# dmosopt/dmosopt

Measured on NVIDIA H100. Metric: candidate-evals/sec (GP+sort+HV) pop=65536 dim=30 obj=3, higher is better.
Workload: dtype f64 results; GP variance contraction in split-fp16 wgmma with fp32 accumulation (precision=auto: calibrated against the float64 path, 0 of 65535 rows of the last step recomputed in float64); ranks on u32 ids

## Files before the change

dmosopt_b200/csrc/gp_tensor.cu:

```cuda
#include <cuda.h>
#include <cuda_fp16.h>
#include <cudaTypedefs.h>
#include <stdlib.h>

#include "gp.cuh"

namespace {

constexpr int TN = 256;
constexpr int TMV = 128;
constexpr int TK = 32;
constexpr int UK = 16;
constexpr int STAGES = 4;
constexpr int A_BYTES = TMV * TK * 2;
constexpr int B_BYTES = TN * TK * 2;
constexpr int STAGE_BYTES = 2 * A_BYTES + 2 * B_BYTES;
constexpr size_t GEMM_SMEM = (size_t)STAGES * STAGE_BYTES + 1024 + 256;
constexpr int NTHREADS = 384;

__device__ __forceinline__ uint32_t smem_u32(const void* p) { return (uint32_t)__cvta_generic_to_shared(p); }

__device__ __forceinline__ void mbar_init(uint64_t* bar, uint32_t count) {
  asm volatile("mbarrier.init.shared::cta.b64 [%0], %1;" ::"r"(smem_u32(bar)), "r"(count) : "memory");
}
__device__ __forceinline__ void mbar_arrive(uint64_t* bar) {
  asm volatile("mbarrier.arrive.shared::cta.b64 _, [%0];" ::"r"(smem_u32(bar)) : "memory");
}
__device__ __forceinline__ void mbar_expect_tx(uint64_t* bar, uint32_t bytes) {
  asm volatile("mbarrier.arrive.expect_tx.shared::cta.b64 _, [%0], %1;" ::"r"(smem_u32(bar)), "r"(bytes) : "memory");
}
__device__ __forceinline__ bool mbar_try_wait(uint64_t* bar, uint32_t parity) {
  uint32_t ok;
  asm volatile(
      "{\n"
      ".reg .pred p;\n"
      "mbarrier.try_wait.parity.shared::cta.b64 p, [%1], %2;\n"
      "selp.u32 %0, 1, 0, p;\n"
      "}\n"
      : "=r"(ok)
      : "r"(smem_u32(bar)), "r"(parity)
      : "memory");
  return ok != 0;
}
__device__ __forceinline__ void mbar_wait(uint64_t* bar, uint32_t parity, volatile int* abort_flag) {
  uint32_t spins = 0;
  while (!mbar_try_wait(bar, parity)) {
    if ((++spins & 0x3FFu) == 0u) {
      if (*abort_flag) return;
      if (spins > (1u << 22)) {
        *abort_flag = 1;
        return;
      }
    }
  }
}

__device__ __forceinline__ void tma_load_2d(const CUtensorMap* map, uint64_t* bar, void* dst, int c0, int c1) {
  asm volatile(
      "cp.async.bulk.tensor.2d.shared::cluster.global.tile.mbarrier::complete_tx::bytes [%0], [%1, {%3, %4}], [%2];" ::"r"(
          smem_u32(dst)),
      "l"(map), "r"(smem_u32(bar)), "r"(c0), "r"(c1)
      : "memory");
}

__device__ __forceinline__ uint64_t make_sdesc64(uint32_t smem_addr) {
  return (uint64_t)((smem_addr >> 4) & 0x3FFFu) | (1ull << 16) | ((uint64_t)(512 >> 4) << 32) | (2ull << 62);
}

__device__ __forceinline__ void wgmma_fence() { asm volatile("wgmma.fence.sync.aligned;" ::: "memory"); }
__device__ __forceinline__ void wgmma_commit() { asm volatile("wgmma.commit_group.sync.aligned;" ::: "memory"); }
template <int N>
__device__ __forceinline__ void wgmma_wait() {
  asm volatile("wgmma.wait_group.sync.aligned %0;" ::"n"(N) : "memory");
}

__device__ __forceinline__ void wgmma_f16_m64n256(float (&d)[128], uint64_t adesc, uint64_t bdesc, uint32_t accumulate) {
  asm volatile(
      "{\n"
      ".reg .pred p;\n"
      "setp.ne.b32 p, %130, 0;\n"
      "wgmma.mma_async.sync.aligned.m64n256k16.f32.f16.f16 "
      "{"
      "%0, %1, %2, %3, %4, %5, %6, %7, %8, %9, %10, %11, %12, %13, %14, %15, "
      "%16, %17, %18, %19, %20, %21, %22, %23, %24, %25, %26, %27, %28, %29, %30, %31, "
      "%32, %33, %34, %35, %36, %37, %38, %39, %40, %41, %42, %43, %44, %45, %46, %47, "
      "%48, %49, %50, %51, %52, %53, %54, %55, %56, %57, %58, %59, %60, %61, %62, %63, "
      "%64, %65, %66, %67, %68, %69, %70, %71, %72, %73, %74, %75, %76, %77, %78, %79, "
      "%80, %81, %82, %83, %84, %85, %86, %87, %88, %89, %90, %91, %92, %93, %94, %95, "
      "%96, %97, %98, %99, %100, %101, %102, %103, %104, %105, %106, %107, %108, %109, %110, %111, "
      "%112, %113, %114, %115, %116, %117, %118, %119, %120, %121, %122, %123, %124, %125, %126, %127}, "
      "%128, %129, p, 1, 1, 0, 0;\n"
      "}\n"
      : "+f"(d[0]), "+f"(d[1]), "+f"(d[2]), "+f"(d[3]), "+f"(d[4]), "+f"(d[5]), "+f"(d[6]), "+f"(d[7]),
        "+f"(d[8]), "+f"(d[9]), "+f"(d[10]), "+f"(d[11]), "+f"(d[12]), "+f"(d[13]), "+f"(d[14]), "+f"(d[15]),
        "+f"(d[16]), "+f"(d[17]), "+f"(d[18]), "+f"(d[19]), "+f"(d[20]), "+f"(d[21]), "+f"(d[22]), "+f"(d[23]),
        "+f"(d[24]), "+f"(d[25]), "+f"(d[26]), "+f"(d[27]), "+f"(d[28]), "+f"(d[29]), "+f"(d[30]), "+f"(d[31]),
        "+f"(d[32]), "+f"(d[33]), "+f"(d[34]), "+f"(d[35]), "+f"(d[36]), "+f"(d[37]), "+f"(d[38]), "+f"(d[39]),
        "+f"(d[40]), "+f"(d[41]), "+f"(d[42]), "+f"(d[43]), "+f"(d[44]), "+f"(d[45]), "+f"(d[46]), "+f"(d[47]),
        "+f"(d[48]), "+f"(d[49]), "+f"(d[50]), "+f"(d[51]), "+f"(d[52]), "+f"(d[53]), "+f"(d[54]), "+f"(d[55]),
        "+f"(d[56]), "+f"(d[57]), "+f"(d[58]), "+f"(d[59]), "+f"(d[60]), "+f"(d[61]), "+f"(d[62]), "+f"(d[63]),
        "+f"(d[64]), "+f"(d[65]), "+f"(d[66]), "+f"(d[67]), "+f"(d[68]), "+f"(d[69]), "+f"(d[70]), "+f"(d[71]),
        "+f"(d[72]), "+f"(d[73]), "+f"(d[74]), "+f"(d[75]), "+f"(d[76]), "+f"(d[77]), "+f"(d[78]), "+f"(d[79]),
        "+f"(d[80]), "+f"(d[81]), "+f"(d[82]), "+f"(d[83]), "+f"(d[84]), "+f"(d[85]), "+f"(d[86]), "+f"(d[87]),
        "+f"(d[88]), "+f"(d[89]), "+f"(d[90]), "+f"(d[91]), "+f"(d[92]), "+f"(d[93]), "+f"(d[94]), "+f"(d[95]),
        "+f"(d[96]), "+f"(d[97]), "+f"(d[98]), "+f"(d[99]), "+f"(d[100]), "+f"(d[101]), "+f"(d[102]), "+f"(d[103]),
        "+f"(d[104]), "+f"(d[105]), "+f"(d[106]), "+f"(d[107]), "+f"(d[108]), "+f"(d[109]), "+f"(d[110]), "+f"(d[111]),
        "+f"(d[112]), "+f"(d[113]), "+f"(d[114]), "+f"(d[115]), "+f"(d[116]), "+f"(d[117]), "+f"(d[118]), "+f"(d[119]),
        "+f"(d[120]), "+f"(d[121]), "+f"(d[122]), "+f"(d[123]), "+f"(d[124]), "+f"(d[125]), "+f"(d[126]), "+f"(d[127])
      : "l"(adesc), "l"(bdesc), "r"(accumulate)
      : "memory");
}

struct GemmParams {
  int M, n_pb, n_jt, n_q;
  int64_t k_rows, l_rows;
  const float* inv_scale;
  double* vnorm;
  int64_t vn_ld;
  int* abort_flag;
};

__device__ __forceinline__ int item_blocks(const GemmParams& p, int q) { return q == p.n_jt - 1 - q ? 1 : 2; }
__device__ __forceinline__ int item_row_block(const GemmParams& p, int q, int s) { return s ? p.n_jt - 1 - q : q; }

__global__ void __launch_bounds__(NTHREADS, 1)
    gp_var_wgmma_kernel(const __grid_constant__ CUtensorMap map_kh, const __grid_constant__ CUtensorMap map_kl,
                        const __grid_constant__ CUtensorMap map_lh, const __grid_constant__ CUtensorMap map_ll,
                        const GemmParams prm) {
  extern __shared__ uint8_t smem_raw[];
  uint8_t* tiles = (uint8_t*)(((uintptr_t)smem_raw + 1023) & ~(uintptr_t)1023);
  uint64_t* bars = (uint64_t*)(tiles + (size_t)STAGES * STAGE_BYTES);
  uint64_t* full = bars;
  uint64_t* empty = bars + STAGES;
  volatile int* abort_flag = prm.abort_flag;
  const int warp = threadIdx.x >> 5, lane = threadIdx.x & 31;

  if (threadIdx.x == 0) {
    for (int s = 0; s < STAGES; ++s) {
      mbar_init(&full[s], 1);
      mbar_init(&empty[s], 8);
    }
    asm volatile("fence.mbarrier_init.release.cluster;" ::: "memory");
  }
  __syncthreads();
  const int per_m = prm.n_pb * prm.n_q;
  const int n_work = prm.M * per_m;

  if (warp >= 8) {
    asm volatile("setmaxnreg.dec.sync.aligned.u32 40;\n" ::: "memory");
    if (warp == 8 && lane == 0) {
      uint32_t stage = 0, phase = 0;
      for (int w = blockIdx.x; w < n_work; w += gridDim.x) {
        const int m = w / per_m, r = w - m * per_m;
        const int pb = r / prm.n_q, q = r - pb * prm.n_q;
        const int a_row = (int)(m * prm.k_rows + (int64_t)pb * TMV);
        const int nb = item_blocks(prm, q);
        for (int s = 0; s < nb; ++s) {
          const int jt = item_row_block(prm, q, s);
          const int b_row = (int)(m * prm.l_rows + (int64_t)jt * TN);
          const int nkc = (jt + 1) * (TN / TK);
          for (int kc = 0; kc < nkc; ++kc) {
            mbar_wait(&empty[stage], phase ^ 1u, abort_flag);
            uint8_t* st = tiles + (size_t)stage * STAGE_BYTES;
            mbar_expect_tx(&full[stage], STAGE_BYTES);
            tma_load_2d(&map_kh, &full[stage], st, kc * TK, a_row);
            tma_load_2d(&map_kl, &full[stage], st + A_BYTES, kc * TK, a_row);
            tma_load_2d(&map_lh, &full[stage], st + 2 * A_BYTES, kc * TK, b_row);
            tma_load_2d(&map_ll, &full[stage], st + 2 * A_BYTES + B_BYTES, kc * TK, b_row);
            if (++stage == STAGES) {
              stage = 0;
              phase ^= 1u;
            }
          }
        }
      }
    }
    return;
  }

  asm volatile("setmaxnreg.inc.sync.aligned.u32 232;\n" ::: "memory");
  const int wg = warp >> 2;
  const int row0 = wg * 64 + (warp & 3) * 16 + (lane >> 2);
  const int col0 = 2 * (lane & 3);
  float acc[128];
  uint32_t stage = 0, phase = 0;
  for (int w = blockIdx.x; w < n_work; w += gridDim.x) {
    const int m = w / per_m, r = w - m * per_m;
    const int pb = r / prm.n_q, q = r - pb * prm.n_q;
    const float* isc = prm.inv_scale + (int64_t)m * prm.l_rows;
    double total0 = 0.0, total1 = 0.0;
    const int nb = item_blocks(prm, q);
    for (int s = 0; s < nb; ++s) {
      const int jt = item_row_block(prm, q, s);
      const int nkc = (jt + 1) * (TN / TK);
      uint32_t prev = 0;
      for (int kc = 0; kc < nkc; ++kc) {
        mbar_wait(&full[stage], phase, abort_flag);
        const uint32_t sa = smem_u32(tiles + (size_t)stage * STAGE_BYTES);
        const uint32_t a_off = wg * (64 * TK * 2);
        const uint64_t a_hi = make_sdesc64(sa + a_off), a_lo = make_sdesc64(sa + A_BYTES + a_off);
        const uint64_t b_hi = make_sdesc64(sa + 2 * A_BYTES), b_lo = make_sdesc64(sa + 2 * A_BYTES + B_BYTES);
        wgmma_fence();
#pragma unroll
        for (int ks = 0; ks < TK / UK; ++ks) {
          const uint64_t adv = (uint64_t)((ks * UK * 2) >> 4);
          wgmma_f16_m64n256(acc, a_hi + adv, b_hi + adv, (kc | ks) ? 1u : 0u);
          wgmma_f16_m64n256(acc, a_hi + adv, b_lo + adv, 1u);
          wgmma_f16_m64n256(acc, a_lo + adv, b_hi + adv, 1u);
        }
        wgmma_commit();
        if (kc > 0) {
          wgmma_wait<1>();
          if (lane == 0) mbar_arrive(&empty[prev]);
        }
        prev = stage;
        if (++stage == STAGES) {
          stage = 0;
          phase ^= 1u;
        }
      }
      wgmma_wait<0>();
      if (lane == 0) mbar_arrive(&empty[prev]);
      const float* sc = isc + jt * TN + col0;
#pragma unroll
      for (int g = 0; g < TN / 32; ++g) {
        float p0[4] = {0.f, 0.f, 0.f, 0.f}, p1[4] = {0.f, 0.f, 0.f, 0.f};
#pragma unroll
        for (int u = 0; u < 4; ++u) {
          const int i = 4 * g + u;
          const float2 sv = __ldg(reinterpret_cast<const float2*>(sc + 8 * i));
          const float t00 = acc[4 * i] * sv.x, t01 = acc[4 * i + 1] * sv.y;
          const float t10 = acc[4 * i + 2] * sv.x, t11 = acc[4 * i + 3] * sv.y;
          p0[u] = fmaf(t01, t01, t00 * t00);
          p1[u] = fmaf(t11, t11, t10 * t10);
        }
        total0 += ((double)p0[0] + (double)p0[1]) + ((double)p0[2] + (double)p0[3]);
        total1 += ((double)p1[0] + (double)p1[1]) + ((double)p1[2] + (double)p1[3]);
      }
    }
#pragma unroll
    for (int o = 1; o < 4; o <<= 1) {
      total0 += __shfl_xor_sync(0xffffffffu, total0, o);
      total1 += __shfl_xor_sync(0xffffffffu, total1, o);
    }
    if ((lane & 3) == 0) {
      const int64_t o = ((int64_t)q * prm.M + m) * prm.vn_ld + (int64_t)pb * TMV + row0;
      prm.vnorm[o] = total0;
      prm.vnorm[o + 8] = total1;
    }
  }
}

__global__ void split_linv_kernel(const double* __restrict__ Linv, int64_t Npad, const int* __restrict__ k_exp,
                                  uint16_t* __restrict__ Lh, uint16_t* __restrict__ Ll, float* __restrict__ inv_scale) {
  const int64_t row = blockIdx.x;
  const int g = (int)(row / Npad);
  const double* src = Linv + row * Npad;
  __shared__ double red[256];
  double mx = 0.0;
  for (int64_t k = threadIdx.x; k < Npad; k += blockDim.x) mx = fmax(mx, fabs(src[k]));
  red[threadIdx.x] = mx;
  __syncthreads();
  for (int o = 128; o > 0; o >>= 1) {
    if (threadIdx.x < o) red[threadIdx.x] = fmax(red[threadIdx.x], red[threadIdx.x + o]);
    __syncthreads();
  }
  mx = red[0];
  int e = 0;
  if (mx > 0.0) e = 13 - ilogb(mx);
  const double s = scalbn(1.0, e);
  for (int64_t k = threadIdx.x; k < Npad; k += blockDim.x) {
    const float x = (float)(src[k] * s);
    const __half h = __float2half_rn(x);
    const __half l = __float2half_rn(x - __half2float(h));
    Lh[row * Npad + k] = __half_as_ushort(h);
    Ll[row * Npad + k] = __half_as_ushort(l);
  }
  if (threadIdx.x == 0) inv_scale[row] = (mx > 0.0) ? (float)scalbn(1.0, -e - k_exp[g]) : 0.f;
}

constexpr int KT_TN = 128, KT_TP = 32;

__device__ __forceinline__ float stationary_f(float s2, int kind) {
  if (kind == DMO_KERNEL_MATERN52) {
    float r;
    asm("sqrt.approx.ftz.f32 %0, %1;" : "=f"(r) : "f"(s2));
    const float K = r * 2.2360679774997896f;
    return fmaf(K, fmaf(K, 1.0f / 3.0f, 1.0f), 1.0f) * __expf(-K);
  }
  return __expf(-0.5f * s2);
}

__device__ __forceinline__ float2 fadd2(float2 a, float2 b) { return make_float2(__fadd_rn(a.x, b.x), __fadd_rn(a.y, b.y)); }
__device__ __forceinline__ float2 fmul2(float2 a, float2 b) { return make_float2(__fmul_rn(a.x, b.x), __fmul_rn(a.y, b.y)); }
__device__ __forceinline__ float2 ffma2(float2 a, float2 b, float2 c) {
  return make_float2(__fmaf_rn(a.x, b.x, c.x), __fmaf_rn(a.y, b.y, c.y));
}

__device__ __forceinline__ float2 stationary2_f(float2 s2, int kind) {
  float2 e;
  if (kind == DMO_KERNEL_MATERN52) {
    float2 r;
    asm("sqrt.approx.ftz.f32 %0, %1;" : "=f"(r.x) : "f"(s2.x));
    asm("sqrt.approx.ftz.f32 %0, %1;" : "=f"(r.y) : "f"(s2.y));
    const float2 K = fmul2(r, make_float2(2.2360679774997896f, 2.2360679774997896f));
    const float2 one = make_float2(1.0f, 1.0f);
    const float2 p = ffma2(K, ffma2(K, make_float2(1.0f / 3.0f, 1.0f / 3.0f), one), one);
    const float2 t = fmul2(K, make_float2(-1.4426950408889634f, -1.4426950408889634f));
    asm("ex2.approx.ftz.f32 %0, %1;" : "=f"(e.x) : "f"(t.x));
    asm("ex2.approx.ftz.f32 %0, %1;" : "=f"(e.y) : "f"(t.y));
    return fmul2(p, e);
  }
  const float2 t = fmul2(s2, make_float2(-0.5f * 1.4426950408889634f, -0.5f * 1.4426950408889634f));
  asm("ex2.approx.ftz.f32 %0, %1;" : "=f"(e.x) : "f"(t.x));
  asm("ex2.approx.ftz.f32 %0, %1;" : "=f"(e.y) : "f"(t.y));
  return e;
}

template <bool ISO, int DMAX>
__global__ void __launch_bounds__(KT_TN)
    kstar_tensor_kernel(const double* __restrict__ Xn, int64_t P, int64_t p_base, int64_t Pcpad,
                        const double* __restrict__ Xt, int64_t N, int d, int M, int kind,
                        const double* __restrict__ inv_ls, const double* __restrict__ constant,
                        const int* __restrict__ k_exp, int64_t ldk, int64_t plane, uint16_t* __restrict__ Kh,
                        uint16_t* __restrict__ Kl) {
  extern __shared__ __align__(16) float sxf[];
  float* s_il = sxf + KT_TP * DMAX;
  float* s_c = s_il + M * DMAX;
  const int64_t n0 = ((int64_t)blockIdx.x * KT_TN + threadIdx.x) * 2;
  const int64_t pt0 = (int64_t)blockIdx.y * KT_TP;
  for (int t = threadIdx.x; t < KT_TP * DMAX; t += KT_TN) {
    const int64_t p = p_base + pt0 + t / DMAX;
    const int j = t % DMAX;
    sxf[t] = (p < P && j < d) ? (float)Xn[p * d + j] : 0.f;
  }
  for (int t = threadIdx.x; t < M * DMAX; t += KT_TN) {
    const int m = t / DMAX, j = t % DMAX;
    s_il[t] = j < d ? (float)inv_ls[m * d + j] : 0.f;
  }
  if (threadIdx.x < M) s_c[threadIdx.x] = scalbnf((float)constant[threadIdx.x], k_exp[threadIdx.x]);
  float2 xa[DMAX / 2], xb[DMAX / 2];
#pragma unroll
  for (int j = 0; j < DMAX / 2; ++j) {
    const int j0 = 2 * j, j1 = 2 * j + 1;
    xa[j] = make_float2((j0 < d && n0 < N) ? (float)Xt[n0 * d + j0] : 0.f, (j1 < d && n0 < N) ? (float)Xt[n0 * d + j1] : 0.f);
    xb[j] = make_float2((j0 < d && n0 + 1 < N) ? (float)Xt[(n0 + 1) * d + j0] : 0.f,
                        (j1 < d && n0 + 1 < N) ? (float)Xt[(n0 + 1) * d + j1] : 0.f);
  }
  __syncthreads();
  const bool live_a = n0 < N, live_b = n0 + 1 < N;
  uint32_t* Kh32 = reinterpret_cast<uint32_t*>(Kh);
  uint32_t* Kl32 = reinterpret_cast<uint32_t*>(Kl);
  for (int q = 0; q < KT_TP; ++q) {
    const int64_t pl = pt0 + q;
    if (pl >= Pcpad || n0 >= ldk) break;
    const float4* xc = reinterpret_cast<const float4*>(sxf + q * DMAX);
    float sa = 0.f, sb = 0.f;
    if (ISO) {
      float2 acc_a0 = make_float2(0.f, 0.f), acc_a1 = acc_a0, acc_b0 = acc_a0, acc_b1 = acc_a0;
#pragma unroll
      for (int j = 0; j < DMAX / 4; ++j) {
        const float4 c = xc[j];
        const float2 c01 = make_float2(c.x, c.y), c23 = make_float2(c.z, c.w);
        const float2 da0 = fadd2(c01, make_float2(-xa[2 * j].x, -xa[2 * j].y));
        const float2 db0 = fadd2(c01, make_float2(-xb[2 * j].x, -xb[2 * j].y));
        const float2 da1 = fadd2(c23, make_float2(-xa[2 * j + 1].x, -xa[2 * j + 1].y));
        const float2 db1 = fadd2(c23, make_float2(-xb[2 * j + 1].x, -xb[2 * j + 1].y));
        acc_a0 = ffma2(da0, da0, acc_a0);
        acc_b0 = ffma2(db0, db0, acc_b0);
        acc_a1 = ffma2(da1, da1, acc_a1);
        acc_b1 = ffma2(db1, db1, acc_b1);
      }
      sa = (acc_a0.x + acc_a0.y) + (acc_a1.x + acc_a1.y);
      sb = (acc_b0.x + acc_b0.y) + (acc_b1.x + acc_b1.y);
    }
    for (int m = 0; m < M; ++m) {
      float2 rr;
      if (ISO) {
        const float il = s_il[m * DMAX];
        const float il2 = il * il;
        rr = fmul2(make_float2(sa, sb), make_float2(il2, il2));
      } else {
        const float4* il4 = reinterpret_cast<const float4*>(s_il + m * DMAX);
        float2 acc_a = make_float2(0.f, 0.f), acc_b = acc_a;
#pragma unroll
        for (int j = 0; j < DMAX / 4; ++j) {
          const float4 c = xc[j], il = il4[j];
          const float2 c01 = make_float2(c.x, c.y), c23 = make_float2(c.z, c.w);
          const float2 i01 = make_float2(il.x, il.y), i23 = make_float2(il.z, il.w);
          const float2 da0 = fmul2(fadd2(c01, make_float2(-xa[2 * j].x, -xa[2 * j].y)), i01);
          const float2 db0 = fmul2(fadd2(c01, make_float2(-xb[2 * j].x, -xb[2 * j].y)), i01);
          const float2 da1 = fmul2(fadd2(c23, make_float2(-xa[2 * j + 1].x, -xa[2 * j + 1].y)), i23);
          const float2 db1 = fmul2(fadd2(c23, make_float2(-xb[2 * j + 1].x, -xb[2 * j + 1].y)), i23);
          acc_a = ffma2(da0, da0, acc_a);
          acc_b = ffma2(db0, db0, acc_b);
          acc_a = ffma2(da1, da1, acc_a);
          acc_b = ffma2(db1, db1, acc_b);
        }
        rr = make_float2(acc_a.x + acc_a.y, acc_b.x + acc_b.y);
      }
      const float sc = s_c[m];
      const float2 kk = fmul2(stationary2_f(rr, kind), make_float2(sc, sc));
      const float ka = live_a ? kk.x : 0.f;
      const float kb = live_b ? kk.y : 0.f;
      const __half2 h = __floats2half2_rn(ka, kb);
      const float2 hf = __half22float2(h);
      const __half2 l = __floats2half2_rn(ka - hf.x, kb - hf.y);
      const int64_t o = (m * plane + pl * ldk + n0) >> 1;
      Kh32[o] = *reinterpret_cast<const uint32_t*>(&h);
      Kl32[o] = *reinterpret_cast<const uint32_t*>(&l);
    }
  }
}

constexpr int KM_T = 128, KM_Q = 256, KM_NS = 32, KM_D = 32;

__global__ void pad_xt_f32_kernel(const double* __restrict__ Xt, int64_t N, int d, int64_t Npad, float* __restrict__ Xtf) {
  const int64_t t = (int64_t)blockIdx.x * blockDim.x + threadIdx.x;
  if (t >= Npad * KM_D) return;
  const int64_t n = t / KM_D;
  const int j = (int)(t % KM_D);
  Xtf[t] = (n < N && j < d) ? (float)Xt[n * d + j] : 0.f;
}

__global__ void pad_calpha_f32_kernel(const double* __restrict__ alpha, const double* __restrict__ constant, int64_t N, int M,
                                      int64_t Npad, float* __restrict__ CAf) {
  const int64_t t = (int64_t)blockIdx.x * blockDim.x + threadIdx.x;
  if (t >= (int64_t)M * Npad) return;
  const int m = (int)(t / Npad);
// ... 346 lines not shown
                                     const int* __restrict__ cov, const double* __restrict__ constant, const double* __restrict__ noise,
                                     const double* __restrict__ ystd, int64_t p_base, double* __restrict__ var) {
  int64_t t = (int64_t)blockIdx.x * blockDim.x + threadIdx.x;
  if (t >= Pc * M) return;
  int64_t pl = t / M;
  int m = (int)(t - pl * M);
  double vn = 0.0;
  const int g = cov[m];
  for (int q = 0; q < nplanes; ++q) vn += vnorm[((int64_t)q * G + g) * ld + pl];
  double v = (constant[m] + noise[m]) - vn;
  if (v < 0.0) v = 0.0;
  double sd = sqrt(v * (ystd[m] * ystd[m]));
  var[(p_base + pl) * M + m] = sd * sd;
}

PFN_cuTensorMapEncodeTiled_v12000 get_encode_fn() {
  static PFN_cuTensorMapEncodeTiled_v12000 fn = nullptr;
  if (!fn) {
    void* p = nullptr;
    cudaDriverEntryPointQueryResult q;
    if (cudaGetDriverEntryPoint("cuTensorMapEncodeTiled", &p, cudaEnableDefault, &q) == cudaSuccess &&
        q == cudaDriverEntryPointSuccess)
      fn = (PFN_cuTensorMapEncodeTiled_v12000)p;
  }
  return fn;
}

int make_map(dmo_ctx* ctx, CUtensorMap* map, const void* base, uint64_t rows, uint64_t cols, uint32_t box_rows,
             uint32_t box_cols, CUtensorMapSwizzle swz) {
  auto fn = get_encode_fn();
  if (!fn) return dmo_fail(ctx, DMO_ERR_CUDA, "cuTensorMapEncodeTiled entry point not available");
  cuuint64_t gdim[2] = {cols, rows};
  cuuint64_t gstr[1] = {cols * 2};
  cuuint32_t box[2] = {box_cols, box_rows};
  cuuint32_t estr[2] = {1, 1};
  CUresult r = fn(map, CU_TENSOR_MAP_DATA_TYPE_FLOAT16, 2, const_cast<void*>(base), gdim, gstr, box, estr,
                  CU_TENSOR_MAP_INTERLEAVE_NONE, swz, CU_TENSOR_MAP_L2_PROMOTION_L2_256B,
                  CU_TENSOR_MAP_FLOAT_OOB_FILL_NONE);
  if (r != CUDA_SUCCESS) return dmo_fail(ctx, DMO_ERR_CUDA, "cuTensorMapEncodeTiled failed with %d", (int)r);
  return DMO_OK;
}

int prepare_direct_state(dmo_ctx* ctx, dmo_gp* gp) {
  if (gp->Xtf.p && gp->CAf.p) return DMO_OK;
  const int64_t N = gp->N, Npad = gp->ops.Npad;
  DMO_TRY(gp->Xtf.alloc(ctx, (size_t)Npad * KM_D));
  DMO_TRY(gp->CAf.alloc(ctx, (size_t)gp->M * Npad));
  DMO_LAUNCH(pad_xt_f32_kernel, (unsigned)ceil_div(Npad * KM_D, 256), 256, 0, gp->Xt.p, N, gp->d, Npad, gp->Xtf.p);
  DMO_LAUNCH(pad_calpha_f32_kernel, (unsigned)ceil_div((int64_t)gp->M * Npad, 256), 256, 0, gp->alpha.p, gp->constant.p, N, gp->M, Npad,
             gp->CAf.p);
  DMO_CHECK_LAUNCH();
  return DMO_OK;
}

int64_t pick_slices(int64_t n_qb, int64_t Npad, int tile, int64_t slots, int64_t* n_per_block) {
  int64_t best = 1;
  double best_eff = -1.0;
  *n_per_block = Npad;
  const int64_t smax = Npad / 256 > 1 ? Npad / 256 : 1;
  for (int64_t sp = 1; sp <= smax; ++sp) {
    const int64_t npb = ceil_div(ceil_div(Npad, sp), (int64_t)tile) * tile;
    const int64_t ns = ceil_div(Npad, npb);
    const int64_t blocks = ns * n_qb;
    const double eff = (double)blocks / (double)(ceil_div(blocks, slots) * slots);
    if (eff > best_eff + 0.02) {
      best_eff = eff;
      best = ns;
      *n_per_block = npb;
    }
  }
  return best;
}

int gp_mean_direct(dmo_ctx* ctx, dmo_gp* gp, const double* dXn, int64_t P, double* d_mean) {
  const int64_t N = gp->N, Npad = gp->ops.Npad;
  const int M = gp->M, d = gp->d;
  DMO_TRY(prepare_direct_state(ctx, gp));
  DevBuf<double> mpart;
  for (int64_t p_base = 0; p_base < P; p_base += GP_MAX_CHUNK) {
    const int64_t Pc = (P - p_base) < GP_MAX_CHUNK ? (P - p_base) : GP_MAX_CHUNK;
    const int64_t n_qb = ceil_div(Pc, KM_Q);
    int64_t n_per_block = Npad;
    const int64_t nsplit = pick_slices(n_qb, Npad, KM_NS, (int64_t)4 * ctx->sm_count, &n_per_block);
    const int64_t ld = n_qb * KM_Q;
    DMO_TRY(mpart.alloc(ctx, (size_t)nsplit * M * ld));
    dim3 grid((unsigned)nsplit, (unsigned)n_qb);
    {
      ProfileScope ps_(ctx, "gp_mean_direct");
#define KM_LAUNCH(ISO_, MT_)                                                                                                  \
  do {                                                                                                                      \
    if (d <= 16)                                                                                                            \
      DMO_LAUNCH((gp_mean_direct_kernel<ISO_, MT_, 4>), grid, KM_T, 0, dXn, P, p_base, gp->Xtf.p, N, Npad, n_per_block,     \
                 d, gp->kernel, gp->inv_ls.p, gp->constant.p, gp->alpha.p, mpart.p, ld);                                    \
    else                                                                                                                    \
      DMO_LAUNCH((gp_mean_direct_kernel<ISO_, MT_, 8>), grid, KM_T, 0, dXn, P, p_base, gp->Xtf.p, N, Npad, n_per_block,     \
                 d, gp->kernel, gp->inv_ls.p, gp->constant.p, gp->alpha.p, mpart.p, ld);                                    \
  } while (0)
#define KM_SWITCH(ISO_)        \
  switch (M) {                 \
    case 1: KM_LAUNCH(ISO_, 1); break; \
    case 2: KM_LAUNCH(ISO_, 2); break; \
    case 3: KM_LAUNCH(ISO_, 3); break; \
    case 4: KM_LAUNCH(ISO_, 4); break; \
    case 5: KM_LAUNCH(ISO_, 5); break; \
    default: KM_LAUNCH(ISO_, 6); break; \
  }
      if (gp->isotropic) {
        KM_SWITCH(true)
      } else {
        KM_SWITCH(false)
      }
#undef KM_SWITCH
#undef KM_LAUNCH
    }
    DMO_LAUNCH(mean_finish_tc_kernel, (unsigned)ceil_div(Pc * M, 256), 256, 0, mpart.p, (int)nsplit, Pc, ld, M, gp->ymean.p,
               gp->ystd.p, p_base, d_mean);
  }
  DMO_CHECK_LAUNCH();
  return DMO_OK;
}

}

int gp_prepare_tensor(dmo_ctx* ctx, GpVarOps& ops) {
  if (ops.tensor_ready) return DMO_OK;
  const int G = ops.G;
  const int64_t Npad = ops.Npad;
  std::vector<int> kexp(G);
  for (int g = 0; g < G; ++g) {
    double c = ops.h_kscale[g];
    kexp[g] = (c > 0.0) ? 13 - ilogb(c) : 13;
  }
  DMO_TRY(ops.Kexp.alloc(ctx, G));
  DMO_CUDA(cudaMemcpyAsync(ops.Kexp.p, kexp.data(), G * sizeof(int), cudaMemcpyHostToDevice, ctx->stream));
  DMO_CUDA(dmo_wait(ctx));
  DMO_TRY(ops.Lhi.alloc(ctx, (size_t)G * Npad * Npad));
  DMO_TRY(ops.Llo.alloc(ctx, (size_t)G * Npad * Npad));
  DMO_TRY(ops.Lscale.alloc(ctx, (size_t)G * Npad));
  DMO_LAUNCH(split_linv_kernel, (unsigned)(G * Npad), 256, 0, ops.Linv.p, Npad, ops.Kexp.p, ops.Lhi.p, ops.Llo.p,
             ops.Lscale.p);
  DMO_CHECK_LAUNCH();
  ops.tensor_ready = true;
  return DMO_OK;
}

static_assert(TMV == GP_TC_TILE, "gp.cuh exports the wgmma candidate tile");

int gp_tensor_var_planes(int64_t Npad) { return (int)((Npad / TN + 1) / 2); }

int gp_var_contract_tensor(dmo_ctx* ctx, const GpVarOps& ops, const uint16_t* Kh, const uint16_t* Kl, int64_t k_alloc,
                           int64_t k_rows, int64_t Pcpad, double* vnorm, int64_t vn_ld, int* abort_flag, int free_sms) {
  const int64_t Npad = ops.Npad;
  DMO_REQUIRE(Npad % TN == 0 && Pcpad % TMV == 0, "gp_var_contract_tensor: internal padding error");
  CUtensorMap map_kh, map_kl, map_lh, map_ll;
  DMO_TRY(make_map(ctx, &map_kh, Kh, (uint64_t)k_alloc, (uint64_t)Npad, TMV, TK, CU_TENSOR_MAP_SWIZZLE_64B));
  DMO_TRY(make_map(ctx, &map_kl, Kl, (uint64_t)k_alloc, (uint64_t)Npad, TMV, TK, CU_TENSOR_MAP_SWIZZLE_64B));
  DMO_TRY(make_map(ctx, &map_lh, ops.Lhi.p, (uint64_t)ops.G * Npad, (uint64_t)Npad, TN, TK, CU_TENSOR_MAP_SWIZZLE_64B));
  DMO_TRY(make_map(ctx, &map_ll, ops.Llo.p, (uint64_t)ops.G * Npad, (uint64_t)Npad, TN, TK, CU_TENSOR_MAP_SWIZZLE_64B));
  DMO_CUDA(cudaFuncSetAttribute(gp_var_wgmma_kernel, cudaFuncAttributeMaxDynamicSharedMemorySize, (int)GEMM_SMEM));
  GemmParams prm;
  prm.M = ops.G;
  prm.n_pb = (int)(Pcpad / TMV);
  prm.n_jt = (int)(Npad / TN);
  prm.n_q = gp_tensor_var_planes(Npad);
  prm.k_rows = k_rows;
  prm.l_rows = Npad;
  prm.inv_scale = ops.Lscale.p;
  prm.vnorm = vnorm;
  prm.vn_ld = vn_ld;
  prm.abort_flag = abort_flag;
  const int n_work = prm.M * prm.n_pb * prm.n_q;
  const int per_cta = (int)ceil_div(n_work, ctx->sm_count - free_sms > 1 ? ctx->sm_count - free_sms : 1);
  const int grid = (int)ceil_div(n_work, per_cta);
  DMO_LAUNCH(gp_var_wgmma_kernel, grid, NTHREADS, GEMM_SMEM, map_kh, map_kl, map_lh, map_ll, prm);
  return DMO_OK;
}

const char* const GP_WATCHDOG_MSG = "gp_predict(tensor): pipeline watchdog tripped (mbarrier wait timed out)";

int gp_predict_tensor(dmo_ctx* ctx, dmo_gp* gp, const double* dXn, int64_t P, double* d_mean, double* d_var, int* abort_flag,
                      const GpOverlap* ov, bool var_route_mean) {
  const int64_t N = gp->N, Npad = gp->ops.Npad;
  const int M = gp->M, G = gp->ops.G, d = gp->d;
  DMO_REQUIRE(M <= 16, "gp_predict(tensor): at most 16 objectives per model (got %d)", M);
  DMO_REQUIRE(d <= 64, "gp_predict(tensor): at most 64 input dimensions (got %d); use DMO_GP_FP64", d);
  DMO_REQUIRE(Npad % TN == 0, "gp_predict(tensor): internal padding error");
  const bool mean_only = !d_var && var_route_mean;
  if (!d_var && !mean_only && d <= KM_D && M <= 6)
    return gp_mean_direct(ctx, gp, dXn, P, d_mean);
  const bool fused = d <= KM_D && M <= 6 && (gp->isotropic || G <= 2) &&
                     !(getenv("DMO_GP_FUSED") && atoi(getenv("DMO_GP_FUSED")) == 0);
  const bool store = !(mean_only && fused);
  if (store) DMO_TRY(gp_prepare_tensor(ctx, gp->ops));
  constexpr int64_t TMv = KM_Q;
  int64_t Pc_max = ((int64_t)6 << 30) / ((int64_t)G * Npad * 4);
  if (Pc_max > GP_MAX_CHUNK) Pc_max = GP_MAX_CHUNK;
  Pc_max = (Pc_max / TMv) * TMv;
  if (Pc_max < TMv) Pc_max = TMv;
  const int64_t Pc_alloc = P < Pc_max ? ceil_div(P, TMv) * TMv : Pc_max;
  const int n_q = gp_tensor_var_planes(Npad);
  DevBuf<uint16_t> Kh, Kl;
  DevBuf<double> vnorm;
  DevBuf<int> own_flag;
  if (store) {
    DMO_TRY(Kh.alloc(ctx, (size_t)G * Pc_alloc * Npad));
    DMO_TRY(Kl.alloc(ctx, (size_t)G * Pc_alloc * Npad));
  }
  const bool read_back = abort_flag == nullptr && !mean_only;
  if (!mean_only) {
    DMO_TRY(vnorm.alloc(ctx, (size_t)n_q * G * Pc_alloc));
    if (read_back) {
      DMO_TRY(own_flag.alloc(ctx, 1));
      abort_flag = own_flag.p;
    }
    DMO_CUDA(cudaMemsetAsync(abort_flag, 0, sizeof(int), ctx->stream));
  }
  const int64_t kplane = Pc_alloc * Npad;
  DevBuf<double> mpart;
  if (fused) DMO_TRY(prepare_direct_state(ctx, gp));
  for (int64_t p_base = 0; p_base < P; p_base += Pc_alloc) {
    const int64_t Pc = (P - p_base) < Pc_alloc ? (P - p_base) : Pc_alloc;
    const int64_t Pcpad = ceil_div(Pc, TMv) * TMv;
    if (fused) {
      int64_t n_per_block = Npad;
      const int64_t n_qb = Pcpad / KM_Q;
      const int64_t nsplit = pick_slices(n_qb, Npad, KF_NS, (int64_t)3 * ctx->sm_count, &n_per_block);
      DMO_TRY(mpart.alloc(ctx, (size_t)nsplit * M * Pcpad));
      dim3 gf((unsigned)nsplit, (unsigned)(Pcpad / KS_Q));
      const size_t smem = kstar_mean_smem(M);
      {
        ProfileScope ps_(ctx, "gp_kstar");
#define KF_LAUNCH_ST(ISO_, MT_, GR_, ST_)                                                                                      \
  do {                                                                                                                          \
    DMO_CUDA(cudaFuncSetAttribute(kstar_mean_kernel<ISO_, MT_, GR_, ST_>, cudaFuncAttributeMaxDynamicSharedMemorySize, (int)smem)); \
    DMO_LAUNCH((kstar_mean_kernel<ISO_, MT_, GR_, ST_>), gf, KS_T, smem, dXn, P, p_base, gp->Xtf.p, N, Npad, n_per_block, d,          \
               gp->kernel, G, gp->cov.p, gp->g_inv_ls.p, gp->g_constant.p, gp->ops.Kexp.p, gp->CAf.p, kplane, Kh.p, Kl.p,        \
               mpart.p, Pcpad);                                                                                                 \
  } while (0)
#define KF_LAUNCH(ISO_, MT_, GR_)            \
  do {                                       \
    if (store)                               \
      KF_LAUNCH_ST(ISO_, MT_, GR_, true);    \
    else                                     \
      KF_LAUNCH_ST(ISO_, MT_, GR_, false);   \
  } while (0)
#define KF_SWITCH(ISO_)                                         \
  if (G < M) {                                                  \
    switch (M) {                                    \
      case 2: KF_LAUNCH(ISO_, 2, true); break;                  \
      case 3: KF_LAUNCH(ISO_, 3, true); break;                  \
      case 4: KF_LAUNCH(ISO_, 4, true); break;                  \
      case 5: KF_LAUNCH(ISO_, 5, true); break;                  \
      default: KF_LAUNCH(ISO_, 6, true); break;                 \
    }                                                           \
  } else {                                                      \
    switch (M) {                                                \
      case 1: KF_LAUNCH(ISO_, 1, false); break;                 \
      case 2: KF_LAUNCH(ISO_, 2, false); break;                 \
      case 3: KF_LAUNCH(ISO_, 3, false); break;                 \
      case 4: KF_LAUNCH(ISO_, 4, false); break;                 \
      case 5: KF_LAUNCH(ISO_, 5, false); break;                 \
      default: KF_LAUNCH(ISO_, 6, false); break;                \
    }                                                           \
  }
        if (gp->isotropic) {
          KF_SWITCH(true)
        } else {
          KF_SWITCH(false)
        }
#undef KF_SWITCH
#undef KF_LAUNCH
#undef KF_LAUNCH_ST
      }
      DMO_LAUNCH(mean_finish_tc_kernel, (unsigned)ceil_div(Pc * M, 256), 256, 0, mpart.p, (int)nsplit, Pc, Pcpad, M, gp->ymean.p,
                 gp->ystd.p, p_base, d_mean);
    } else {
      {
        ProfileScope ps_(ctx, "gp_kstar");
        const int dmax = d <= 32 ? 32 : 64;
        size_t smem = (size_t)(KT_TP * dmax + G * dmax + G) * sizeof(float);
        dim3 gk((unsigned)(Npad / (2 * KT_TN)), (unsigned)ceil_div(Pcpad, KT_TP));
#define KSTAR_LAUNCH(ISO_, DM_)                                                                                          \
  DMO_LAUNCH((kstar_tensor_kernel<ISO_, DM_>), gk, KT_TN, smem, dXn, P, p_base, Pcpad, gp->Xt.p, N, d, G, gp->kernel, \
             gp->g_inv_ls.p, gp->g_constant.p, gp->ops.Kexp.p, Npad, kplane, Kh.p, Kl.p)
        if (gp->isotropic) {
          if (d <= 32)
            KSTAR_LAUNCH(true, 32);
          else
            KSTAR_LAUNCH(true, 64);
        } else {
          if (d <= 32)
            KSTAR_LAUNCH(false, 32);
          else
            KSTAR_LAUNCH(false, 64);
        }
#undef KSTAR_LAUNCH
      }
      {
        ProfileScope ps_(ctx, "gp_mean");
        DMO_LAUNCH(mean_split_kernel, (unsigned)ceil_div(Pc * M * 32, 256), 256, 0, Kh.p, Kl.p, Pc, N, Npad, kplane, M,
                   gp->cov.p, gp->ops.Kexp.p, gp->alpha.p, gp->ymean.p, gp->ystd.p, p_base, d_mean);
      }
    }
    if (ov && p_base + Pc_alloc >= P) DMO_CUDA(cudaEventRecord(ov->mean_ready, ctx->stream));
    if (d_var) {
      {
        ProfileScope ps_(ctx, "gp_var");
        cudaStream_t main = ctx->stream;
        if (ov) {
          DMO_CUDA(cudaEventRecord(ctx->lane_ev[1], main));
          DMO_CUDA(cudaStreamWaitEvent(ctx->gp_hi, ctx->lane_ev[1], 0));
          ctx->stream = ctx->gp_hi;
        }
        const int rc = gp_var_contract_tensor(ctx, gp->ops, Kh.p, Kl.p, G * Pc_alloc, Pc_alloc, Pcpad, vnorm.p, Pc_alloc, abort_flag,
                                              ov ? GP_LANE_SMS : 0);
        if (ov) {
          ctx->stream = main;
          DMO_CUDA(cudaEventRecord(ctx->lane_ev[2], ctx->gp_hi));
          DMO_CUDA(cudaStreamWaitEvent(main, ctx->lane_ev[2], 0));
        }
        DMO_TRY(rc);
      }
      DMO_LAUNCH(var_finish_tc_kernel, (unsigned)ceil_div(Pc * M, 256), 256, 0, vnorm.p, n_q, Pc, Pc_alloc, M, G,
                 gp->cov.p, gp->constant.p, gp->noise.p, gp->ystd.p, p_base, d_var);
    }
  }
  DMO_CHECK_LAUNCH();
// ... 8 lines not shown
```

Measured before the change: 9.293 million.

## Skip zero upper-triangle of L^-1 in diagonal tiles via narrower wgmma

Reverses the row order of the split L-inverse planes within each 256-row tile so that, on diagonal k-chunks, the zero triangular part sits at the end of the N dimension. Per-chunk TMA maps with shrinking row counts load only the nonzero rows, and wgmma variants with smaller N (256 down to 16) skip the zero columns. The epilogue remaps accumulator indices and scale columns to undo the reversal. This cuts tensor-core work and L traffic on diagonal blocks, at the cost of 16 TMA descriptors, a larger kernel parameter block, a switch over 8 templated paths, and more fragile indexing.

```diff
diff --git a/dmosopt_b200/csrc/gp_tensor.cu b/dmosopt_b200/csrc/gp_tensor.cu
--- a/dmosopt_b200/csrc/gp_tensor.cu
+++ b/dmosopt_b200/csrc/gp_tensor.cu
@@ -74,42 +74,72 @@
   asm volatile("wgmma.wait_group.sync.aligned %0;" ::"n"(N) : "memory");
 }
 
-__device__ __forceinline__ void wgmma_f16_m64n256(float (&d)[128], uint64_t adesc, uint64_t bdesc, uint32_t accumulate) {
-  asm volatile(
-      "{\n"
-      ".reg .pred p;\n"
-      "setp.ne.b32 p, %130, 0;\n"
-      "wgmma.mma_async.sync.aligned.m64n256k16.f32.f16.f16 "
-      "{"
-      "%0, %1, %2, %3, %4, %5, %6, %7, %8, %9, %10, %11, %12, %13, %14, %15, "
-      "%16, %17, %18, %19, %20, %21, %22, %23, %24, %25, %26, %27, %28, %29, %30, %31, "
-      "%32, %33, %34, %35, %36, %37, %38, %39, %40, %41, %42, %43, %44, %45, %46, %47, "
-      "%48, %49, %50, %51, %52, %53, %54, %55, %56, %57, %58, %59, %60, %61, %62, %63, "
-      "%64, %65, %66, %67, %68, %69, %70, %71, %72, %73, %74, %75, %76, %77, %78, %79, "
-      "%80, %81, %82, %83, %84, %85, %86, %87, %88, %89, %90, %91, %92, %93, %94, %95, "
-      "%96, %97, %98, %99, %100, %101, %102, %103, %104, %105, %106, %107, %108, %109, %110, %111, "
-      "%112, %113, %114, %115, %116, %117, %118, %119, %120, %121, %122, %123, %124, %125, %126, %127}, "
-      "%128, %129, p, 1, 1, 0, 0;\n"
-      "}\n"
-      : "+f"(d[0]), "+f"(d[1]), "+f"(d[2]), "+f"(d[3]), "+f"(d[4]), "+f"(d[5]), "+f"(d[6]), "+f"(d[7]),
-        "+f"(d[8]), "+f"(d[9]), "+f"(d[10]), "+f"(d[11]), "+f"(d[12]), "+f"(d[13]), "+f"(d[14]), "+f"(d[15]),
-        "+f"(d[16]), "+f"(d[17]), "+f"(d[18]), "+f"(d[19]), "+f"(d[20]), "+f"(d[21]), "+f"(d[22]), "+f"(d[23]),
-        "+f"(d[24]), "+f"(d[25]), "+f"(d[26]), "+f"(d[27]), "+f"(d[28]), "+f"(d[29]), "+f"(d[30]), "+f"(d[31]),
-        "+f"(d[32]), "+f"(d[33]), "+f"(d[34]), "+f"(d[35]), "+f"(d[36]), "+f"(d[37]), "+f"(d[38]), "+f"(d[39]),
-        "+f"(d[40]), "+f"(d[41]), "+f"(d[42]), "+f"(d[43]), "+f"(d[44]), "+f"(d[45]), "+f"(d[46]), "+f"(d[47]),
-        "+f"(d[48]), "+f"(d[49]), "+f"(d[50]), "+f"(d[51]), "+f"(d[52]), "+f"(d[53]), "+f"(d[54]), "+f"(d[55]),
-        "+f"(d[56]), "+f"(d[57]), "+f"(d[58]), "+f"(d[59]), "+f"(d[60]), "+f"(d[61]), "+f"(d[62]), "+f"(d[63]),
-        "+f"(d[64]), "+f"(d[65]), "+f"(d[66]), "+f"(d[67]), "+f"(d[68]), "+f"(d[69]), "+f"(d[70]), "+f"(d[71]),
-        "+f"(d[72]), "+f"(d[73]), "+f"(d[74]), "+f"(d[75]), "+f"(d[76]), "+f"(d[77]), "+f"(d[78]), "+f"(d[79]),
-        "+f"(d[80]), "+f"(d[81]), "+f"(d[82]), "+f"(d[83]), "+f"(d[84]), "+f"(d[85]), "+f"(d[86]), "+f"(d[87]),
-        "+f"(d[88]), "+f"(d[89]), "+f"(d[90]), "+f"(d[91]), "+f"(d[92]), "+f"(d[93]), "+f"(d[94]), "+f"(d[95]),
-        "+f"(d[96]), "+f"(d[97]), "+f"(d[98]), "+f"(d[99]), "+f"(d[100]), "+f"(d[101]), "+f"(d[102]), "+f"(d[103]),
-        "+f"(d[104]), "+f"(d[105]), "+f"(d[106]), "+f"(d[107]), "+f"(d[108]), "+f"(d[109]), "+f"(d[110]), "+f"(d[111]),
-        "+f"(d[112]), "+f"(d[113]), "+f"(d[114]), "+f"(d[115]), "+f"(d[116]), "+f"(d[117]), "+f"(d[118]), "+f"(d[119]),
-        "+f"(d[120]), "+f"(d[121]), "+f"(d[122]), "+f"(d[123]), "+f"(d[124]), "+f"(d[125]), "+f"(d[126]), "+f"(d[127])
-      : "l"(adesc), "l"(bdesc), "r"(accumulate)
-      : "memory");
-}
+#define WG_LIST_15 "%0, %1, %2, %3, %4, %5, %6, %7"
+#define WG_LIST_14 WG_LIST_15 ", %8, %9, %10, %11, %12, %13, %14, %15"
+#define WG_LIST_13 WG_LIST_14 ", %16, %17, %18, %19, %20, %21, %22, %23"
+#define WG_LIST_12 WG_LIST_13 ", %24, %25, %26, %27, %28, %29, %30, %31"
+#define WG_LIST_11 WG_LIST_12 ", %32, %33, %34, %35, %36, %37, %38, %39"
+#define WG_LIST_10 WG_LIST_11 ", %40, %41, %42, %43, %44, %45, %46, %47"
+#define WG_LIST_9 WG_LIST_10 ", %48, %49, %50, %51, %52, %53, %54, %55"
+#define WG_LIST_8 WG_LIST_9 ", %56, %57, %58, %59, %60, %61, %62, %63"
+#define WG_LIST_7 WG_LIST_8 ", %64, %65, %66, %67, %68, %69, %70, %71"
+#define WG_LIST_6 WG_LIST_7 ", %72, %73, %74, %75, %76, %77, %78, %79"
+#define WG_LIST_5 WG_LIST_6 ", %80, %81, %82, %83, %84, %85, %86, %87"
+#define WG_LIST_4 WG_LIST_5 ", %88, %89, %90, %91, %92, %93, %94, %95"
+#define WG_LIST_3 WG_LIST_4 ", %96, %97, %98, %99, %100, %101, %102, %103"
+#define WG_LIST_2 WG_LIST_3 ", %104, %105, %106, %107, %108, %109, %110, %111"
+#define WG_LIST_1 WG_LIST_2 ", %112, %113, %114, %115, %116, %117, %118, %119"
+#define WG_LIST_0 WG_LIST_1 ", %120, %121, %122, %123, %124, %125, %126, %127"
+#define WG_ACC_OPERANDS(d)                                                                                              \
+  "+f"(d[0]), "+f"(d[1]), "+f"(d[2]), "+f"(d[3]), "+f"(d[4]), "+f"(d[5]), "+f"(d[6]), "+f"(d[7]),                       \
+  "+f"(d[8]), "+f"(d[9]), "+f"(d[10]), "+f"(d[11]), "+f"(d[12]), "+f"(d[13]), "+f"(d[14]), "+f"(d[15]),                 \
+  "+f"(d[16]), "+f"(d[17]), "+f"(d[18]), "+f"(d[19]), "+f"(d[20]), "+f"(d[21]), "+f"(d[22]), "+f"(d[23]),               \
+  "+f"(d[24]), "+f"(d[25]), "+f"(d[26]), "+f"(d[27]), "+f"(d[28]), "+f"(d[29]), "+f"(d[30]), "+f"(d[31]),               \
+  "+f"(d[32]), "+f"(d[33]), "+f"(d[34]), "+f"(d[35]), "+f"(d[36]), "+f"(d[37]), "+f"(d[38]), "+f"(d[39]),               \
+  "+f"(d[40]), "+f"(d[41]), "+f"(d[42]), "+f"(d[43]), "+f"(d[44]), "+f"(d[45]), "+f"(d[46]), "+f"(d[47]),               \
+  "+f"(d[48]), "+f"(d[49]), "+f"(d[50]), "+f"(d[51]), "+f"(d[52]), "+f"(d[53]), "+f"(d[54]), "+f"(d[55]),               \
+  "+f"(d[56]), "+f"(d[57]), "+f"(d[58]), "+f"(d[59]), "+f"(d[60]), "+f"(d[61]), "+f"(d[62]), "+f"(d[63]),               \
+  "+f"(d[64]), "+f"(d[65]), "+f"(d[66]), "+f"(d[67]), "+f"(d[68]), "+f"(d[69]), "+f"(d[70]), "+f"(d[71]),               \
+  "+f"(d[72]), "+f"(d[73]), "+f"(d[74]), "+f"(d[75]), "+f"(d[76]), "+f"(d[77]), "+f"(d[78]), "+f"(d[79]),               \
+  "+f"(d[80]), "+f"(d[81]), "+f"(d[82]), "+f"(d[83]), "+f"(d[84]), "+f"(d[85]), "+f"(d[86]), "+f"(d[87]),               \
+  "+f"(d[88]), "+f"(d[89]), "+f"(d[90]), "+f"(d[91]), "+f"(d[92]), "+f"(d[93]), "+f"(d[94]), "+f"(d[95]),               \
+  "+f"(d[96]), "+f"(d[97]), "+f"(d[98]), "+f"(d[99]), "+f"(d[100]), "+f"(d[101]), "+f"(d[102]), "+f"(d[103]),           \
+  "+f"(d[104]), "+f"(d[105]), "+f"(d[106]), "+f"(d[107]), "+f"(d[108]), "+f"(d[109]), "+f"(d[110]), "+f"(d[111]),       \
+  "+f"(d[112]), "+f"(d[113]), "+f"(d[114]), "+f"(d[115]), "+f"(d[116]), "+f"(d[117]), "+f"(d[118]), "+f"(d[119]),       \
+  "+f"(d[120]), "+f"(d[121]), "+f"(d[122]), "+f"(d[123]), "+f"(d[124]), "+f"(d[125]), "+f"(d[126]), "+f"(d[127])
+
+template <int T>
+__device__ __forceinline__ void wgmma_f16(float (&d)[128], uint64_t adesc, uint64_t bdesc, uint32_t accumulate);
+#define WGMMA_F16(T, N)                                                                                                   \
+  template <>                                                                                                            \
+  __device__ __forceinline__ void wgmma_f16<T>(float (&d)[128], uint64_t adesc, uint64_t bdesc, uint32_t accumulate) {  \
+    static_assert(N == 256 - 16 * T, "wgmma N");                                                                          \
+    asm volatile("{\n"                                                                                                    \
+                 ".reg .pred p;\n"                                                                                        \
+                 "setp.ne.b32 p, %130, 0;\n"                                                                              \
+                 "wgmma.mma_async.sync.aligned.m64n" #N "k16.f32.f16.f16 {" WG_LIST_##T "}, %128, %129, p, 1, 1, 0, 0;\n" \
+                 "}\n"                                                                                                    \
+                 : WG_ACC_OPERANDS(d)                                                                                     \
+                 : "l"(adesc), "l"(bdesc), "r"(accumulate)                                                                \
+                 : "memory");                                                                                             \
+  }
+WGMMA_F16(0, 256)
+WGMMA_F16(1, 240)
+WGMMA_F16(2, 224)
+WGMMA_F16(3, 208)
+WGMMA_F16(4, 192)
+WGMMA_F16(5, 176)
+WGMMA_F16(6, 160)
+WGMMA_F16(7, 144)
+WGMMA_F16(8, 128)
+WGMMA_F16(9, 112)
+WGMMA_F16(10, 96)
+WGMMA_F16(11, 80)
+WGMMA_F16(12, 64)
+WGMMA_F16(13, 48)
+WGMMA_F16(14, 32)
+WGMMA_F16(15, 16)
+#undef WGMMA_F16
 
 struct GemmParams {
   int M, n_pb, n_jt, n_q;
@@ -123,10 +153,31 @@
 __device__ __forceinline__ int item_blocks(const GemmParams& p, int q) { return q == p.n_jt - 1 - q ? 1 : 2; }
 __device__ __forceinline__ int item_row_block(const GemmParams& p, int q, int s) { return s ? p.n_jt - 1 - q : q; }
 
+struct LinvMaps {
+  CUtensorMap hi[TN / TK], lo[TN / TK];
+};
+
+template <int T>
+__device__ __forceinline__ void mma_k16(float (&acc)[128], uint64_t a_hi, uint64_t a_lo, uint64_t b_hi, uint64_t b_lo,
+                                        uint32_t accumulate) {
+  wgmma_f16<T>(acc, a_hi, b_hi, accumulate);
+  wgmma_f16<T>(acc, a_hi, b_lo, 1u);
+  wgmma_f16<T>(acc, a_lo, b_hi, 1u);
+}
+
+template <int T0, int T1>
+__device__ __forceinline__ void mma_chunk(float (&acc)[128], uint64_t a_hi, uint64_t a_lo, uint64_t b_hi, uint64_t b_lo,
+                                          uint32_t accumulate) {
+  constexpr uint64_t adv = (UK * 2) >> 4;
+  wgmma_fence();
+  mma_k16<T0>(acc, a_hi, a_lo, b_hi, b_lo, accumulate);
+  mma_k16<T1>(acc, a_hi + adv, a_lo + adv, b_hi + adv, b_lo + adv, 1u);
+  wgmma_commit();
+}
+
 __global__ void __launch_bounds__(NTHREADS, 1)
     gp_var_wgmma_kernel(const __grid_constant__ CUtensorMap map_kh, const __grid_constant__ CUtensorMap map_kl,
-                        const __grid_constant__ CUtensorMap map_lh, const __grid_constant__ CUtensorMap map_ll,
-                        const GemmParams prm) {
+                        const __grid_constant__ LinvMaps lmaps, const GemmParams prm) {
   extern __shared__ uint8_t smem_raw[];
   uint8_t* tiles = (uint8_t*)(((uintptr_t)smem_raw + 1023) & ~(uintptr_t)1023);
   uint64_t* bars = (uint64_t*)(tiles + (size_t)STAGES * STAGE_BYTES);
@@ -160,13 +211,15 @@
           const int b_row = (int)(m * prm.l_rows + (int64_t)jt * TN);
           const int nkc = (jt + 1) * (TN / TK);
           for (int kc = 0; kc < nkc; ++kc) {
+            const int c = kc - jt * (TN / TK) > 0 ? kc - jt * (TN / TK) : 0;
+            const int r0 = TK * c;
             mbar_wait(&empty[stage], phase ^ 1u, abort_flag);
             uint8_t* st = tiles + (size_t)stage * STAGE_BYTES;
-            mbar_expect_tx(&full[stage], STAGE_BYTES);
+            mbar_expect_tx(&full[stage], 2 * A_BYTES + 2 * (TN - r0) * TK * 2);
             tma_load_2d(&map_kh, &full[stage], st, kc * TK, a_row);
             tma_load_2d(&map_kl, &full[stage], st + A_BYTES, kc * TK, a_row);
-            tma_load_2d(&map_lh, &full[stage], st + 2 * A_BYTES, kc * TK, b_row);
-            tma_load_2d(&map_ll, &full[stage], st + 2 * A_BYTES + B_BYTES, kc * TK, b_row);
+            tma_load_2d(&lmaps.hi[c], &full[stage], st + 2 * A_BYTES, kc * TK, b_row);
+            tma_load_2d(&lmaps.lo[c], &full[stage], st + 2 * A_BYTES + B_BYTES, kc * TK, b_row);
             if (++stage == STAGES) {
               stage = 0;
               phase ^= 1u;
@@ -181,7 +234,7 @@
   asm volatile("setmaxnreg.inc.sync.aligned.u32 232;\n" ::: "memory");
   const int wg = warp >> 2;
   const int row0 = wg * 64 + (warp & 3) * 16 + (lane >> 2);
-  const int col0 = 2 * (lane & 3);
+  const int lr = 2 * (3 - (lane & 3));
   float acc[128];
   uint32_t stage = 0, phase = 0;
   for (int w = blockIdx.x; w < n_work; w += gridDim.x) {
@@ -200,15 +253,18 @@
         const uint32_t a_off = wg * (64 * TK * 2);
         const uint64_t a_hi = make_sdesc64(sa + a_off), a_lo = make_sdesc64(sa + A_BYTES + a_off);
         const uint64_t b_hi = make_sdesc64(sa + 2 * A_BYTES), b_lo = make_sdesc64(sa + 2 * A_BYTES + B_BYTES);
-        wgmma_fence();
-#pragma unroll
-        for (int ks = 0; ks < TK / UK; ++ks) {
-          const uint64_t adv = (uint64_t)((ks * UK * 2) >> 4);
-          wgmma_f16_m64n256(acc, a_hi + adv, b_hi + adv, (kc | ks) ? 1u : 0u);
-          wgmma_f16_m64n256(acc, a_hi + adv, b_lo + adv, 1u);
-          wgmma_f16_m64n256(acc, a_lo + adv, b_hi + adv, 1u);
-        }
-        wgmma_commit();
+        const uint32_t accumulate = kc ? 1u : 0u;
+        switch (kc - jt * (TN / TK)) {
+          case 0: mma_chunk<0, 1>(acc, a_hi, a_lo, b_hi, b_lo, accumulate); break;
+          case 1: mma_chunk<2, 3>(acc, a_hi, a_lo, b_hi, b_lo, accumulate); break;
+          case 2: mma_chunk<4, 5>(acc, a_hi, a_lo, b_hi, b_lo, accumulate); break;
+          case 3: mma_chunk<6, 7>(acc, a_hi, a_lo, b_hi, b_lo, accumulate); break;
+          case 4: mma_chunk<8, 9>(acc, a_hi, a_lo, b_hi, b_lo, accumulate); break;
+          case 5: mma_chunk<10, 11>(acc, a_hi, a_lo, b_hi, b_lo, accumulate); break;
+          case 6: mma_chunk<12, 13>(acc, a_hi, a_lo, b_hi, b_lo, accumulate); break;
+          case 7: mma_chunk<14, 15>(acc, a_hi, a_lo, b_hi, b_lo, accumulate); break;
+          default: mma_chunk<0, 0>(acc, a_hi, a_lo, b_hi, b_lo, accumulate); break;
+        }
         if (kc > 0) {
           wgmma_wait<1>();
           if (lane == 0) mbar_arrive(&empty[prev]);
@@ -221,16 +277,16 @@
       }
       wgmma_wait<0>();
       if (lane == 0) mbar_arrive(&empty[prev]);
-      const float* sc = isc + jt * TN + col0;
+      const float* sc = isc + jt * TN + lr;
 #pragma unroll
       for (int g = 0; g < TN / 32; ++g) {
         float p0[4] = {0.f, 0.f, 0.f, 0.f}, p1[4] = {0.f, 0.f, 0.f, 0.f};
 #pragma unroll
         for (int u = 0; u < 4; ++u) {
-          const int i = 4 * g + u;
+          const int i = 4 * g + u, ir = TN / 8 - 1 - i;
           const float2 sv = __ldg(reinterpret_cast<const float2*>(sc + 8 * i));
-          const float t00 = acc[4 * i] * sv.x, t01 = acc[4 * i + 1] * sv.y;
-          const float t10 = acc[4 * i + 2] * sv.x, t11 = acc[4 * i + 3] * sv.y;
+          const float t00 = acc[4 * ir + 1] * sv.x, t01 = acc[4 * ir] * sv.y;
+          const float t10 = acc[4 * ir + 3] * sv.x, t11 = acc[4 * ir + 2] * sv.y;
           p0[u] = fmaf(t01, t01, t00 * t00);
           p1[u] = fmaf(t11, t11, t10 * t10);
         }
@@ -273,8 +329,8 @@
     const float x = (float)(src[k] * s);
     const __half h = __float2half_rn(x);
     const __half l = __float2half_rn(x - __half2float(h));
-    Lh[row * Npad + k] = __half_as_ushort(h);
-    Ll[row * Npad + k] = __half_as_ushort(l);
+    Lh[(row ^ (TN - 1)) * Npad + k] = __half_as_ushort(h);
+    Ll[(row ^ (TN - 1)) * Npad + k] = __half_as_ushort(l);
   }
   if (threadIdx.x == 0) inv_scale[row] = (mx > 0.0) ? (float)scalbn(1.0, -e - k_exp[g]) : 0.f;
 }
@@ -927,11 +983,15 @@
                            int64_t k_rows, int64_t Pcpad, double* vnorm, int64_t vn_ld, int* abort_flag, int free_sms) {
   const int64_t Npad = ops.Npad;
   DMO_REQUIRE(Npad % TN == 0 && Pcpad % TMV == 0, "gp_var_contract_tensor: internal padding error");
-  CUtensorMap map_kh, map_kl, map_lh, map_ll;
+  CUtensorMap map_kh, map_kl;
+  LinvMaps lmaps;
   DMO_TRY(make_map(ctx, &map_kh, Kh, (uint64_t)k_alloc, (uint64_t)Npad, TMV, TK, CU_TENSOR_MAP_SWIZZLE_64B));
   DMO_TRY(make_map(ctx, &map_kl, Kl, (uint64_t)k_alloc, (uint64_t)Npad, TMV, TK, CU_TENSOR_MAP_SWIZZLE_64B));
-  DMO_TRY(make_map(ctx, &map_lh, ops.Lhi.p, (uint64_t)ops.G * Npad, (uint64_t)Npad, TN, TK, CU_TENSOR_MAP_SWIZZLE_64B));
-  DMO_TRY(make_map(ctx, &map_ll, ops.Llo.p, (uint64_t)ops.G * Npad, (uint64_t)Npad, TN, TK, CU_TENSOR_MAP_SWIZZLE_64B));
+  for (int c = 0; c < TN / TK; ++c) {
+    const uint32_t rows = TN - TK * c;
+    DMO_TRY(make_map(ctx, &lmaps.hi[c], ops.Lhi.p, (uint64_t)ops.G * Npad, (uint64_t)Npad, rows, TK, CU_TENSOR_MAP_SWIZZLE_64B));
+    DMO_TRY(make_map(ctx, &lmaps.lo[c], ops.Llo.p, (uint64_t)ops.G * Npad, (uint64_t)Npad, rows, TK, CU_TENSOR_MAP_SWIZZLE_64B));
+  }
   DMO_CUDA(cudaFuncSetAttribute(gp_var_wgmma_kernel, cudaFuncAttributeMaxDynamicSharedMemorySize, (int)GEMM_SMEM));
   GemmParams prm;
   prm.M = ops.G;
@@ -947,7 +1007,7 @@
   const int n_work = prm.M * prm.n_pb * prm.n_q;
   const int per_cta = (int)ceil_div(n_work, ctx->sm_count - free_sms > 1 ? ctx->sm_count - free_sms : 1);
   const int grid = (int)ceil_div(n_work, per_cta);
-  DMO_LAUNCH(gp_var_wgmma_kernel, grid, NTHREADS, GEMM_SMEM, map_kh, map_kl, map_lh, map_ll, prm);
+  DMO_LAUNCH(gp_var_wgmma_kernel, grid, NTHREADS, GEMM_SMEM, map_kh, map_kl, lmaps, prm);
   return DMO_OK;
 }
 
```

After: 9.503 million (median of 6 runs). +2.3%, better.
